# Princic-1837592/julia-raytracer

Hardware: AMD Instinct MI355X
Metric: Mrays/s + wall-clock render time, cornellbox 1280×720×256spp (higher is better)
Workload: dtype f32; 1 GPU; cornellbox path 1280x720x256spp; scene=cornellbox, sampler=path, width=1280, height=720, spp=256, bounces=8, batch=256, traversal=near, traversal_requested=auto, bvh=middle, parallelism=1 tile groups x 1 sample ranges + RCCL reduce

## Files before the change

### julia-raytracer_amd/csrc/jt_kernels.h

```cpp
#pragma once

#include <hip/hip_runtime.h>

#include <algorithm>

#include "jt_integrator.h"
#include "jt_launch.h"

namespace jtk {
using namespace jtd;

#ifndef JT_STAMPS
#define JT_STAMPS 0
#endif
#ifndef JT_NODE_REPEAT_NONE
#define JT_NODE_REPEAT_NONE 4
#endif
#ifndef JT_NODE_REPEAT
#define JT_NODE_REPEAT 3
#endif
#ifndef JT_FIRST_POP_NONE
#define JT_FIRST_POP_NONE 1
#endif
#ifndef JT_FIRST_POP
#define JT_FIRST_POP 2
#endif
template <int F>
constexpr int first_pops() { return !ft_none(F) && (F & FT_LINL) ? JT_FIRST_POP : JT_FIRST_POP_NONE; }
#ifndef JT_VOTE_P
#define JT_VOTE_P 3
#endif
#ifndef JT_VOTE_N
#define JT_VOTE_N 1
#endif
#ifndef JT_RAY_FROM_PATH
#define JT_RAY_FROM_PATH 1
#endif

__device__ __forceinline__ int lane_count(unsigned long long m) {
    return __builtin_popcount((unsigned)m) + __builtin_popcount((unsigned)(m >> 32));
}

__device__ __forceinline__ unsigned wave_sum(unsigned v) {
    for (int off = 32; off > 0; off >>= 1) v += __shfl_xor(v, off, 64);
    return v;
}

#ifndef JT_KARG_RELOAD
#define JT_KARG_RELOAD 1
#endif
template <int F>
__host__ __device__ constexpr bool karg_reload() {
    return JT_KARG_RELOAD && !mesh_env_quad_family(F);
}
template <class T>
__device__ __forceinline__ T karg(size_t off) {
    typedef __attribute__((address_space(4))) const char* kptr;
    kptr p = (kptr)__builtin_amdgcn_kernarg_segment_ptr();
    asm volatile("" : "+s"(p));
    return *(const __attribute__((address_space(4))) T*)(p + off);
}
#ifndef JT_KARG_SCENE
#define JT_KARG_SCENE 1
#endif
template <bool NCACHE, int F>
__host__ __device__ constexpr bool karg_scene() {
    return NCACHE && JT_KARG_SCENE && !mesh_family(F);
}
template <bool FROM_KARG>
__device__ __forceinline__ const DScene& shade_scene(const DScene& S) {
    if constexpr (FROM_KARG) {
        typedef __attribute__((address_space(4))) const char* kptr;
        kptr p = (kptr)__builtin_amdgcn_kernarg_segment_ptr();
        asm volatile("" : "+s"(p));
        return *(const DScene*)(const __attribute__((address_space(4))) DScene*)(p + offsetof(KArgs, S));
    } else {
        return S;
    }
}
#ifndef JT_KARG_PARAMS
#define JT_KARG_PARAMS 1
#endif
template <int SAMPLER, int F>
__host__ __device__ constexpr bool karg_params_on() {
    return JT_KARG_PARAMS && SAMPLER == 1 && !mesh_family(F);
}
template <bool FROM_KARG>
__device__ __forceinline__ const DParams& karg_params(const DParams& P) {
    if constexpr (FROM_KARG) {
        typedef __attribute__((address_space(4))) const char* kptr;
        kptr p = (kptr)__builtin_amdgcn_kernarg_segment_ptr();
        asm volatile("" : "+s"(p));
        return *(const DParams*)(const __attribute__((address_space(4))) DParams*)(p + offsetof(KArgs, P));
    } else {
        return P;
    }
}
#ifndef JT_KARG_SCENE_LDS
#define JT_KARG_SCENE_LDS 1
#endif
__device__ __forceinline__ DScene blob_scene(const DScene& S, const uint4* blob);
template <bool NCACHE, int RING, bool OVF, int F>
__device__ __forceinline__ DScene shade_scene_lds(const DScene& S0) {
    if constexpr (!NCACHE && JT_KARG_SCENE_LDS) {
        extern __shared__ uint4 dyn_lds[];
        const DScene& K = shade_scene<true>(S0);
        return blob_scene(K, dyn_lds + lds_stack_bytes(OVF, RING, K.stack_need) / 16);
    } else {
        return S0;
    }
}
#define JT_A(f) (karg_reload<F>() ? karg<decltype(DAccum::f)>(offsetof(KArgs, A) + offsetof(DAccum, f)) : A.f)
#define JT_SB (karg_reload<F>() ? karg<int>(offsetof(KArgs, s_begin)) : s_begin)
#define JT_SE (karg_reload<F>() ? karg<int>(offsetof(KArgs, s_end)) : s_end)


#ifndef JT_BAND_STRIP
#define JT_BAND_STRIP 16
#endif

#ifndef JT_ITEM_FIRST_POP
#define JT_ITEM_FIRST_POP 2
#endif
template <bool WIDE, int F>
__host__ __device__ constexpr bool item_first_pop() {
    return JT_ITEM_FIRST_POP == 1 || (JT_ITEM_FIRST_POP == 2 && !WIDE && !ft_none(F));
}
#ifndef JT_ITEM_COORDS
#define JT_ITEM_COORDS 1
#endif
template <int F>
__host__ __device__ constexpr bool item_coords() {
    return JT_ITEM_COORDS && !mesh_env_quad_family(F);
}
__device__ __forceinline__ int item_pixel(unsigned item, const DParams& P, int tiles_x) {
    const int t = (int)(item >> 6), l = (int)(item & 63u);
    return ((t / tiles_x) * 8 + (l >> 3)) * P.width + (t % tiles_x) * 8 + (l & 7);
}
template <int F>
__device__ __forceinline__ unsigned item_of(int ut, int l, int i, int j) {
    return item_coords<F>() ? item_encode(i, j) : (unsigned)(ut * 64 + l);
}
template <int F>
__device__ __forceinline__ int item_pixel_index(unsigned item, const DParams& P, int tiles_x) {
    return item_coords<F>() ? item_j(item) * P.width + item_i(item) : item_pixel(item, P, tiles_x);
}
template <int F>
__device__ __forceinline__ int item_slot(unsigned item, const DParams& P) {
    if constexpr (item_coords<F>()) return item_slot(item, (P.width + 7) >> 3, P.tile_offset, P.tile_stride_rcp);
    else {
        const float inv = __uint_as_float(__builtin_amdgcn_readfirstlane(__float_as_uint(1.0f / (float)P.tile_stride)));
        return launch_tile((int)(item >> 6), P.tile_offset, inv) * 64 + (int)(item & 63u);
    }
}
__device__ __forceinline__ float stream_weight(const DParams& P, int s) {
    return jl_rcp_weight((float)(((s - P.first) >> P.lk) + 1));
}

#if JT_STAMPS
#define JT_STAMP(x) x
#else
#define JT_STAMP(x)
#endif

template <int SAMPLER, int RING, bool OVF, int COUNT, int F, bool NCACHE, bool WIDE, bool ADAPT = false>
__device__ __forceinline__ void trace_body_items(const DScene& S0, const DParams& P0, int s_begin, int s_end,
                                                 const DAccum& A, int* stack) {
    const DScene& S = S0;
    const DParams& P = P0;
    static_assert(lane_lds(F), "the per-lane item body keeps the lane's sample index in LDS");
    constexpr int PB = push_bit(node_baked<OVF, NCACHE, WIDE, F>());
    const int lane = threadIdx.x & 63;
    const int oslot = (int)blockIdx.x * BLOCK + (int)threadIdx.x;
    if constexpr ((F & (FT_TEX | FT_ENV)) != 0) {
        for (int k = threadIdx.x; k < 512; k += BLOCK) tex_lut[k] = k < 256 ? S.srgb_lut[k] : S.byte_lut[k - 256];
        __syncthreads();
    }
    Counters cnt{0, 0, 0, 0};
    constexpr bool WC = !ft_none(F);
    unsigned w_paths = 0, w_rays = 0, w_lq = 0;
    __shared__ unsigned wave_cnt[WC ? 1 : (BLOCK / 64) * 4];
    unsigned* const wcnt = wave_cnt + (WC ? 0 : (threadIdx.x >> 6) * 4);
    if (!WC && lane < 3) wcnt[lane] = 0u;
    auto lds_count = [&](int k, bool c) {
        if (c) __hip_atomic_fetch_add(wcnt + k, 1u, __ATOMIC_RELAXED, __HIP_MEMORY_SCOPE_WORKGROUP);
    };
    __shared__ float acc_lds[acc_slots(F) * BLOCK];
    float* acc = acc_lds + threadIdx.x;
    int* const acc_i = reinterpret_cast<int*>(acc);
#if JT_STAMPS
    unsigned long long t_trav = 0, t_shade = 0, n_trav = 0, n_shade = 0, lanes_p = 0, lanes_n = 0, steps_p = 0, steps_n = 0;
    unsigned long long t_hit = 0, t_fin = 0, t_qb = 0, n_phit = 0, n_fin = 0, idle = 0, n_mph = 0, n_mty = 0, n_mid = 0;
    unsigned long long lanes_sh = 0, lanes_hit = 0, t_start = 0, n_start = 0, lanes_start = 0;
#endif
    const int tiles_x = (P.width + 7) / 8, tiles = launch_tiles(P);
    const int kstr = 1 << P.lk;
    const int nq = s_end - s_begin < kstr ? s_end - s_begin : kstr;
    unsigned xcc;
    asm volatile("s_getreg_b32 %0, hwreg(HW_REG_XCC_ID)" : "=s"(xcc));
    int band_k = 0;
    int ut = 0, uq = 0, bnext = 64;
    bool drained = false;
    unsigned item = ITEM_NONE;
    bool next_sample = false;
    Aov aov{acc, 0.0f, P.first, P.lk};
    Path st;
    st.pk = acc + acc_base_slots(F) * BLOCK;
    Trav T;
    T.sp = -1;
    T.nprim = 0;
    T.nxt = W_EMPTY;
    for (;;) {
        JT_STAMP(const unsigned long long ts0 = __builtin_amdgcn_s_memtime());
        bool start = next_sample;
        for (;;) {
            const unsigned long long needm = __builtin_amdgcn_ballot_w64(item == ITEM_NONE);
            if (!needm || drained) break;
            if (bnext >= 64) {
                const int band = (int)((xcc + (unsigned)band_k) & (NBANDS - 1));
                constexpr int STRIP = JT_BAND_STRIP;
                const int gx = tiles_x % P.tile_stride == 0 ? tiles_x / P.tile_stride : 0;
                const bool strips = STRIP > 1 && gx > 0;
                const int tiles_y = (P.height + 7) / 8;
                const int bt0 = strips ? band * tiles_y / NBANDS * gx : band * tiles / NBANDS;
                const int bn = strips ? (band + 1) * tiles_y / NBANDS * gx - bt0 : (band + 1) * tiles / NBANDS - bt0;
                unsigned unit = 0;
                if (lane == 0) unit = atomicAdd(JT_A(work) + band * BAND_STRIDE, 1u);
                unit = __builtin_amdgcn_readfirstlane(unit);
                if (unit >= (unsigned)bn * (unsigned)nq) {
                    if (++band_k >= NBANDS) drained = true;
                    continue;
                }
                uq = (int)(unit % (unsigned)nq);
                const int tu = (int)(unit / (unsigned)nq);
                int tile = bt0 + tu;
                if (strips) {
                    const int rows = bn / gx, sidx = tu / (STRIP * gx);
                    const int v = tu - sidx * STRIP * gx, h = rows - sidx * STRIP < STRIP ? rows - sidx * STRIP : STRIP;
                    tile = bt0 + (sidx * STRIP + v % h) * gx + v / h;
                }
                ut = tile * P.tile_stride + P.tile_offset;
                if constexpr (ADAPT) {
                    if (JT_A(frozen)[ut]) {
                        bnext = 64;
                        continue;
                    }
                }
                bnext = 0;
            }
            const int nneed = lane_count(needm), take = nneed < 64 - bnext ? nneed : 64 - bnext;
            const int rank = (int)__builtin_amdgcn_mbcnt_hi((unsigned)(needm >> 32), __builtin_amdgcn_mbcnt_lo((unsigned)needm, 0u));
            if (item == ITEM_NONE && rank < take) {
                const int l = bnext + rank;
                const int i = (ut % tiles_x) * 8 + (l & 7), j = (ut / tiles_x) * 8 + (l >> 3);
                if (i < P.width && j < P.height) {
                    item = item_of<F>(ut, l, i, j);
                    start = true;
                    const int s = JT_SB + uq;
                    acc_i[11 * BLOCK] = s;
                    const int pixel = j * P.width + i;
                    float4 im = make_float4(0, 0, 0, 0), al = im, nr = im;
                    int h = 0;
                    if (s - P.first >= kstr) {
                        if (P.lk == 0) {
                            im = JT_A(image)[pixel];
                            al = JT_A(albedo)[pixel];
                            nr = JT_A(normal)[pixel];
                            h = (int)JT_A(hits)[pixel];
                        } else {
                            const size_t o = (size_t)((s - P.first) & (kstr - 1)) * (size_t)JT_A(nslot) +
                                             (size_t)item_slot<F>(item, P);
                            im = JT_A(part_img)[o];
                            al = JT_A(part_alb)[o];
                            nr = JT_A(part_nrm)[o];
                            h = __float_as_int(al.w);
                        }
                    }
                    acc[0] = im.x;
                    acc[BLOCK] = im.y;
                    acc[2 * BLOCK] = im.z;
                    acc[3 * BLOCK] = im.w;
                    acc[4 * BLOCK] = al.x;
                    acc[5 * BLOCK] = al.y;
                    acc[6 * BLOCK] = al.z;
                    acc[7 * BLOCK] = nr.x;
                    acc[8 * BLOCK] = nr.y;
                    acc[9 * BLOCK] = nr.z;
                    acc_i[10 * BLOCK] = h;
                }
            }
            bnext += take;
        }
        next_sample = false;
        if (start) {
            const int sample = acc_i[11 * BLOCK];
            const int tpixel = item_coords<F>() ? 0 : item_pixel(item, P, tiles_x);
            if (!ft_none(F)) acc[12 * BLOCK] = stream_weight(P, sample);
            const DParams& P = karg_params<karg_params_on<SAMPLER, F>()>(P0);
            const int i = item_coords<F>() ? item_i(item) : tpixel % P.width;
            const int j = item_coords<F>() ? item_j(item) : tpixel / P.width;
            start_path<F>(P, i, j, item_coords<F>() ? j * P.width + i : tpixel, sample, st);
            query_start<WIDE>(S, T, st.o, st.d, -1, stack, 0, PB);
            if (!WC) lds_count(1, true);
            if constexpr (item_first_pop<WIDE, F>()) {
#pragma unroll
                for (int k = 0; k < first_pops<F>(); k++)
                    if (wants_node<WIDE>(T)) node_step_any<WIDE, RING, OVF, COUNT, NCACHE, F>(S, T, stack, oslot, cnt);
            }
        }
        if (WC) w_rays += lane_count(__builtin_amdgcn_ballot_w64(start));
#if JT_STAMPS
        const unsigned long long ts1 = __builtin_amdgcn_s_memtime();
        t_start += ts1 - ts0;
        n_start++;
        lanes_start += lane_count(__builtin_amdgcn_ballot_w64(start));
#endif
        if (__builtin_amdgcn_ballot_w64(item != ITEM_NONE) == 0) break;
        constexpr bool LSTEP = light_steps(SAMPLER, F);
        for (;;) {
            const bool wantp = T.nprim > 0;
            const bool wantn = wants_node<WIDE>(T);
            const bool waiting = query_done<WIDE>(T);
            const int np = lane_count(__builtin_amdgcn_ballot_w64(wantp));
            const int nn = lane_count(__builtin_amdgcn_ballot_w64(wantn));
            int nw = lane_count(__builtin_amdgcn_ballot_w64(waiting));
            const int nb = np + nn;
            if (LSTEP && !S.light_inline) {
                const bool wantl = waiting && st.phase == PH_LIGHT;
                const int nl = lane_count(__builtin_amdgcn_ballot_w64(wantl));
                if (nl > 0 && (nl >= P.light_lanes || nb == 0)) {
                    bool c_lq = false, c_ray = false;
                    if (wantl && rerun_tie<WIDE>(S, T, st.o, st.d, S.lights[st.li].instance, stack, PB)) {
                    } else if (wantl) {
                        if (light_hit<F>(S, P, st, query_hit(T))) {
                            st.phase = PH_FINISH;
                        } else if (st.phase == PH_LIGHT) {
                            if (WC) c_lq = true;
                            else lds_count(2, true);
                            query_start<WIDE>(S, T, st.o, st.d, S.lights[st.li].instance, stack, 0, PB);
                        } else {
                            if (WC) c_ray = true;
                            else lds_count(1, true);
                            query_start<WIDE>(S, T, st.o, st.d, -1, stack, 0, PB);
                        }
                    }
                    if (WC) {
                        w_lq += lane_count(__builtin_amdgcn_ballot_w64(c_lq));
                        w_rays += lane_count(__builtin_amdgcn_ballot_w64(c_ray));
                    }
                    continue;
                }
                nw -= nl;
            }
            if (nb == 0 || nw >= (nb + nw < P.wait_lanes ? nb + nw : P.wait_lanes)) break;
#if JT_STAMPS
            n_trav++;
            idle += 64 - lane_count(__builtin_amdgcn_ballot_w64(item != ITEM_NONE));
            if (np * JT_VOTE_P >= nn * JT_VOTE_N) { steps_p++; lanes_p += np; } else { steps_n++; lanes_n += nn; }
#endif
            if (JT_RAY_FROM_PATH && !(F & FT_XFORM)) {
                T.lo = st.o;
                T.ld = st.d;
            }
            if (np * JT_VOTE_P >= nn * JT_VOTE_N) {
                if (T.nprim > 0) prim_step<COUNT, F>(S, T, cnt);
            } else {
                constexpr int NREP = ft_none(F) ? JT_NODE_REPEAT_NONE : JT_NODE_REPEAT;
#pragma unroll
                for (int k = 0; k < NREP; k++)
                    if (wants_node<WIDE>(T)) node_step_any<WIDE, RING, OVF, COUNT, NCACHE, F>(S, T, stack, oslot, cnt);
            }
        }
#if JT_STAMPS
        const unsigned long long ts2 = __builtin_amdgcn_s_memtime();
        t_trav += ts2 - ts1;
        n_shade++;
        lanes_sh += lane_count(__builtin_amdgcn_ballot_w64(query_done<WIDE>(T)));
        {
            int mid = -1, mt = -1;
            if (query_done<WIDE>(T) && st.phase == PH_SCENE && T.h_inst >= 0) {
                mid = S.inst_shade[T.h_inst].material;
                mt = (F & FT_MAT) ? S.materials[mid].type : (int)M_MATTE;
            }
            if (__builtin_amdgcn_ballot_w64(mt >= 0)) {
                n_mph++;
                lanes_hit += lane_count(__builtin_amdgcn_ballot_w64(mt >= 0));
                for (int ty = 0; ty <= (int)M_GLTFPBR; ty++) n_mty += __builtin_amdgcn_ballot_w64(mt == ty) ? 1u : 0u;
                bool counted = mt < 0;
                for (;;) {
                    const unsigned long long m = __builtin_amdgcn_ballot_w64(!counted);
                    if (!m) break;
                    const int v = __shfl(mid, __ffsll((long long)m) - 1);
                    counted = counted || mid == v;
                    n_mid++;
                }
            }
        }
        unsigned long long ts3 = ts2, ts4 = ts2;
#endif
        constexpr bool LINL = (F & (FT_LINL | FT_NOIL)) != 0;
        {
            const bool tie = query_done<WIDE>(T) && (T.nh & (TIE_SEEN | REF_RERUN)) == TIE_SEEN &&
                             !(LSTEP && st.phase == PH_FINISH);
            if (S.order_flip && __builtin_amdgcn_ballot_w64(tie))
                if (tie) rerun_tie<WIDE>(S, T, st.o, st.d, SAMPLER == 1 && !LINL && st.phase == PH_LIGHT ? S.lights[st.li].instance : -1, stack, PB);
        }
        bool c_path = false, c_lq = false, c_ray = false;
        unsigned n_inl = 0;
        if (query_done<WIDE>(T)) {
            const DParams& P = karg_params<karg_params_on<SAMPLER, F>()>(P0);
            const DScene SL = shade_scene_lds<NCACHE, RING, OVF, F>(S0);
            const DScene& S = NCACHE ? shade_scene<karg_scene<NCACHE, F>()>(S0) : SL;
            bool alive = true;
            const bool light = SAMPLER == 1 && !LINL && st.phase == PH_LIGHT;
            bool done;
            if (LSTEP && st.phase == PH_FINISH) done = true;
            else if (light) done = light_hit<F>(S, P, st, query_hit(T));
            else if (SAMPLER == 2) done = naive_hit<F>(S, P, st, query_hit(T), aov, cnt.shades);
            else done = path_hit<F>(S, P, st, query_hit(T), aov, cnt.shades);
            bool chained = false;
            if (SAMPLER == 1 && !done && st.phase == PH_LIGHT && chains_inline(F, S)) {
                unsigned nlq = 0;
                chained = true;
                done = light_chain<WIDE, RING, OVF, COUNT, NCACHE, F>(S, P, st, T, stack, oslot, cnt, [&] {
                    if (WC) nlq++;
                    else lds_count(2, true);
                });
                if (WC) n_inl += nlq;
            }
#if JT_STAMPS
            ts3 = __builtin_amdgcn_s_memtime();
            n_phit++;
#endif
            if (done) {
                if (WC) c_path = true;
                else lds_count(0, true);
                v3 radiance = st.radiance<F>();
                if (!all_finite(radiance)) radiance = V3(0, 0, 0);
                const float mr = max3(radiance);
                if (mr > P.clamp) radiance = radiance * (P.clamp / mr);
                const float w = aov.w<F>();
                const float omw = 1 - w;
                const bool hit = st.flag(F_HIT);
                const bool env = !hit && !P.envhidden && S.nenvs != 0;
                const v4 target = (hit || env) ? V4(radiance.x, radiance.y, radiance.z, 1) : V4(0, 0, 0, 0);
                if (!hit) aov_update<F>(aov, env ? V3(1, 1, 1) : V3(0, 0, 0), -st.d);
                acc[0] = acc[0] * omw + target.x * w;
                acc[BLOCK] = acc[BLOCK] * omw + target.y * w;
                acc[2 * BLOCK] = acc[2 * BLOCK] * omw + target.z * w;
                acc[3 * BLOCK] = acc[3 * BLOCK] * omw + target.w * w;
                if (hit || env) acc_i[10 * BLOCK] += 1;
                alive = false;
                T.sp = -1;
                const int sample = acc_i[11 * BLOCK];
                if (sample + kstr >= JT_SE) {
                    const int pixel = item_pixel_index<F>(item, P, tiles_x);
                    const float4 im = make_float4(acc[0], acc[BLOCK], acc[2 * BLOCK], acc[3 * BLOCK]);
                    if (P.lk == 0) {
                        JT_A(image)[pixel] = im;
                        JT_A(albedo)[pixel] = make_float4(acc[4 * BLOCK], acc[5 * BLOCK], acc[6 * BLOCK], 0.0f);
                        JT_A(normal)[pixel] = make_float4(acc[7 * BLOCK], acc[8 * BLOCK], acc[9 * BLOCK], 0.0f);
                        JT_A(hits)[pixel] = (long long)acc_i[10 * BLOCK];
                    } else {
                        const size_t o = (size_t)((sample - P.first) & (kstr - 1)) * (size_t)JT_A(nslot) +
                                         (size_t)item_slot<F>(item, P);
                        JT_A(part_img)[o] = im;
                        JT_A(part_alb)[o] = make_float4(acc[4 * BLOCK], acc[5 * BLOCK], acc[6 * BLOCK], __int_as_float(acc_i[10 * BLOCK]));
                        JT_A(part_nrm)[o] = make_float4(acc[7 * BLOCK], acc[8 * BLOCK], acc[9 * BLOCK], 0.0f);
                    }
                    item = ITEM_NONE;
                } else {
                    acc_i[11 * BLOCK] = sample + kstr;
                    next_sample = true;
                }
            }
#if JT_STAMPS
            ts4 = __builtin_amdgcn_s_memtime();
            if (__builtin_amdgcn_ballot_w64(done)) n_fin++;
#endif
            if (alive) {
                if (SAMPLER == 1 && !LINL && st.phase == PH_LIGHT) {
                    if (WC) c_lq = true;
                    else lds_count(2, true);
                    query_start<WIDE>(S, T, st.o, st.d, S.lights[st.li].instance, stack, 0, PB);
                } else {
                    if (WC) c_ray = true;
                    else lds_count(1, true);
                    if (SAMPLER == 1 && chain_dinv_once<WIDE, OVF, NCACHE, F>() && __builtin_amdgcn_ballot_w64(!chained) == 0)
                        query_restart<F>(S, T, st.o, st.d, stack, PB);
                    else query_start<WIDE>(S, T, st.o, st.d, -1, stack, 0, PB);
                }
#pragma unroll
                for (int k = 0; k < first_pops<F>(); k++)
                    if (wants_node<WIDE>(T)) node_step_any<WIDE, RING, OVF, COUNT, NCACHE, F>(S, T, stack, oslot, cnt);
            }
        }
#if JT_STAMPS
        const unsigned long long ts5 = __builtin_amdgcn_s_memtime();
        t_shade += ts5 - ts2;
        t_hit += ts3 - ts2;
        t_fin += ts4 - ts3;
        t_qb += ts5 - ts4;
#endif
        if (WC) {
            w_paths += lane_count(__builtin_amdgcn_ballot_w64(c_path));
            w_lq += lane_count(__builtin_amdgcn_ballot_w64(c_lq));
            w_rays += lane_count(__builtin_amdgcn_ballot_w64(c_ray));
            if (SAMPLER == 1 && chains_inline(F, S)) w_lq += __builtin_amdgcn_readfirstlane(wave_sum(n_inl));
        }
    }
#if JT_STAMPS
    if (lane == 0) {
        unsigned long long* dbg = A.counters + 8;
        const unsigned long long v[24] = {t_trav, t_shade, n_trav,  n_shade, lanes_p, lanes_n,  steps_p, steps_n,
                                          0,      t_hit,   t_fin,   t_qb,    0,       n_phit,   n_fin,   idle,
                                          n_mph,  n_mty,   n_mid,   lanes_sh, lanes_hit, t_start, n_start, lanes_start};
        for (int k = 0; k < 24; k++) atomicAdd(dbg + k, v[k]);
    }
#endif
    const unsigned wv[3] = {w_paths, w_rays, w_lq};
    unsigned v[7] = {0u, 0u, 0u, cnt.nodes, cnt.instances, cnt.prims, COUNT ? cnt.shades : 0u};
#pragma unroll
    for (int k = 0; k < 7; k++) {
        unsigned sum = k < 3 ? (WC ? wv[k] : wcnt[k]) : wave_sum(v[k]);
        if (lane == 0 && sum) atomicAdd(&A.counters[k], (unsigned long long)sum);
    }
}

#ifndef JT_WAVES
#define JT_WAVES 0
#endif
#ifndef JT_WAVES_NONE
#define JT_WAVES_NONE 5
#endif
#if JT_WAVES > 0
#define JT_WAVES_PER_EU __attribute__((amdgpu_waves_per_eu(JT_WAVES, JT_WAVES)))
#define JT_WAVES_PER_EU_F(F) \
    __attribute__((amdgpu_waves_per_eu(ft_none(F) ? JT_WAVES_NONE : JT_WAVES, ft_none(F) ? JT_WAVES_NONE : JT_WAVES)))
#else
#define JT_WAVES_PER_EU
#define JT_WAVES_PER_EU_F(F)
#endif

__device__ __forceinline__ DScene blob_scene(const DScene& S, const uint4* blob) {
    DScene L = S;
    L.nodes = reinterpret_cast<const DNode*>(blob + S.o_nodes);
    L.wnodes = reinterpret_cast<const DWide*>(blob + S.o_wnodes);
    L.prims = reinterpret_cast<const float4*>(blob + S.o_prims);
    L.inst_trav = reinterpret_cast<const DInstTrav*>(blob + S.o_inst_trav);
    L.inst_blas = reinterpret_cast<const int4*>(blob + S.o_inst_blas);
    L.inst_shade = reinterpret_cast<const DInstShade*>(blob + S.o_inst_shade);
    L.shapes = reinterpret_cast<const DShape*>(blob + S.o_shapes);
    L.pos = reinterpret_cast<const float4*>(blob + S.o_pos);
    L.nrm = reinterpret_cast<const float4*>(blob + S.o_nrm);
    L.tc = reinterpret_cast<const float2*>(blob + S.o_tc);
    L.col = reinterpret_cast<const float4*>(blob + S.o_col);
    L.elems = reinterpret_cast<const int4*>(blob + S.o_elems);
    L.enrm = reinterpret_cast<const float4*>(blob + S.o_enrm);
    L.enrm_id = reinterpret_cast<const float4*>(blob + S.o_enrm_id);
    L.materials = reinterpret_cast<const DMaterial*>(blob + S.o_materials);
    L.lights = reinterpret_cast<const DLight*>(blob + S.o_lights);
    L.light_hit = reinterpret_cast<const int4*>(blob + S.o_light_hit);
    L.light_elems = reinterpret_cast<const float4*>(blob + S.o_light_elems);
    L.cdf = reinterpret_cast<const float*>(blob + S.o_cdf);
    return L;
}

__device__ __forceinline__ void bake_nodes(const DScene& S, uint4* blob) {
    uint4* const nodes = blob + S.o_nodes;
    const int nnodes = (S.o_wnodes - S.o_nodes) >> 1;
    for (int k = threadIdx.x; k < nnodes; k += BLOCK) {
        uint4& b = nodes[2 * k + 1];
        const BakedNode bn = bake_node(b.w, (int)b.z, k < S.tlas_nnodes ? T_TLAS : T_BLAS);
        b.z = bn.e0;
        b.w = bn.meta;
    }
}

template <int SAMPLER, int RING, bool OVF, int COUNT, int F, bool WIDE, bool ADAPT>
__global__ __launch_bounds__(BLOCK) JT_WAVES_PER_EU void trace_kernel(DScene S, DParams P, int s_begin, int s_end, DAccum A) {
    __shared__ int lds_stack[RING * BLOCK];
    trace_body_items<SAMPLER, RING, OVF, COUNT, F, true, WIDE, ADAPT>(S, P, s_begin, s_end, A, lds_stack + threadIdx.x);
}

template <int SAMPLER, int RING, bool OVF, int COUNT, int F, bool WIDE, bool ADAPT>
__global__ __launch_bounds__(BLOCK) JT_WAVES_PER_EU_F(F) void trace_kernel_lds(DScene S, DParams P, int s_begin, int s_end, DAccum A) {
    extern __shared__ uint4 dyn_lds[];
    uint4* blob = dyn_lds + lds_stack_bytes(OVF, RING, S.stack_need) / 16;
    for (int k = threadIdx.x; k < S.blob_n16; k += BLOCK) blob[k] = S.blob[k];
    __syncthreads();
    if constexpr (node_baked<OVF, false, WIDE, F>()) {
        bake_nodes(S, blob);
        __syncthreads();
    }
    const DScene L = blob_scene(S, blob);
    trace_body_items<SAMPLER, RING, OVF, COUNT, F, false, WIDE, ADAPT>(L, P, s_begin, s_end, A, reinterpret_cast<int*>(dyn_lds) + threadIdx.x);
}

template <int SAMPLER, int RING, bool OVF, int COUNT, int F, bool LDSK, bool WIDE, bool ADAPT>
hipError_t launch_t(const DScene& S, const DParams& P, int s0, int s1, const DAccum& A, hipStream_t st, int cus) {
    const long long units = (long long)launch_tiles(P) * std::min(s1 - s0, 1 << P.lk);
    const int want = (int)std::min<long long>((units + BLOCK / 64 - 1) / (BLOCK / 64), 1 << 30);
    if (want == 0) return hipSuccess;
    int per_cu = 0;
    hipError_t e;
    if constexpr (LDSK) {
        if (S.blob_n16 > 0) {
        const size_t lds = lds_stack_bytes(OVF, RING, S.stack_need) + (size_t)S.blob_n16 * 16;
        constexpr auto kl = &trace_kernel_lds<SAMPLER, RING, OVF, COUNT, F, WIDE, ADAPT>;
        const void* k = (const void*)kl;
        if ((e = hipFuncSetAttribute(k, hipFuncAttributeMaxDynamicSharedMemorySize, (int)lds)) != hipSuccess) return e;
        if (hipOccupancyMaxActiveBlocksPerMultiprocessor(&per_cu, k, BLOCK, lds) != hipSuccess || per_cu < 1) per_cu = 1;
        const int nwg = std::min(want, std::min(per_cu, 8) * cus);
        hipLaunchKernelGGL(kl, dim3(nwg), dim3(BLOCK), lds, st, S, P, s0, s1, A);
        return hipGetLastError();
        }
    }
    constexpr auto kh = &trace_kernel<SAMPLER, RING, OVF, COUNT, F, WIDE, ADAPT>;
    const void* k = (const void*)kh;
    if (hipOccupancyMaxActiveBlocksPerMultiprocessor(&per_cu, k, BLOCK, 0) != hipSuccess || per_cu < 1) per_cu = 1;
    const int nwg = std::min(want, std::min(per_cu, 8) * cus);
    hipLaunchKernelGGL(kh, dim3(nwg), dim3(BLOCK), 0, st, S, P, s0, s1, A);
    return hipGetLastError();
}

template <int ID, int SAMPLER, int COUNT, bool ADAPT>
hipError_t launch_cfg(const DScene& S, const DParams& P, int s0, int s1, const DAccum& A, hipStream_t st, int cus) {
    using C = LaunchConfig<ID>;
    return launch_t<SAMPLER, C::ring, C::ovf, COUNT, C::feat, C::lds, C::wide, ADAPT>(S, P, s0, s1, A, st, cus);
}

}
```

### julia-raytracer_amd/csrc/jt_push.h

```cpp
#pragma once

#if defined(__HIPCC__) || defined(__CUDACC__)
#define JT_PUSH_HD __host__ __device__ inline
#else
#define JT_PUSH_HD inline
#endif

namespace jtk {

constexpr int PUSH_SLOTS = 4;
constexpr unsigned PUSH_T_INST = 1u, PUSH_SNAP_NONE = 63u << 24;

struct PushPlan {
    int npush;
    int first, step;
    unsigned tag;
    bool leaf;
    int slot[PUSH_SLOTS];
    unsigned value[PUSH_SLOTS];
};

JT_PUSH_HD PushPlan push_plan(unsigned meta, int start, unsigned type, bool blas, int negmask, int sp) {
    PushPlan p;
    const bool internal = (meta >> 24) != 0;
    const int num = (int)(meta & 0xffffu);
    const bool neg = ((negmask >> (int)((meta >> 16) & 3u)) & 1) != 0;
    p.npush = internal ? 2 : blas ? 0 : num;
    p.first = internal ? (neg ? start + 1 : start) : start + num - 1;
    p.step = internal && !neg ? 1 : -1;
    p.tag = (internal ? type << 30 : PUSH_T_INST << 30) | PUSH_SNAP_NONE;
    p.leaf = blas && !internal;
    const int last = (p.npush > 1 ? p.npush : 1) - 1;
    const unsigned e0 = p.tag | (unsigned)p.first;
    for (int j = 0; j < PUSH_SLOTS; j++) {
        const int k = j < last ? j : last;
        p.slot[j] = sp + k;
        p.value[j] = e0 + (unsigned)(p.step * k);
    }
    return p;
}

constexpr unsigned BAKE_AXIS_SET = 3u;
constexpr int BAKE_MASK_BIT = 8;
constexpr unsigned BAKE_LEAF = 1u << 27;

struct BakedNode {
    unsigned e0, meta;
};
JT_PUSH_HD BakedNode bake_node(unsigned meta, int start, unsigned level) {
    const bool internal = (meta >> 24) != 0;
    const bool blas = level != 0u;
    const unsigned num = meta & 0xffffu;
    const unsigned tag = (internal ? level << 30 : PUSH_T_INST << 30) | PUSH_SNAP_NONE;
    const unsigned npush = internal ? 2u : blas ? 0u : (num < (unsigned)PUSH_SLOTS ? num : (unsigned)PUSH_SLOTS);
    const unsigned last = (npush > 1u ? npush : 1u) - 1u;
    BakedNode b;
    b.e0 = internal || !blas ? tag | (unsigned)start : (unsigned)start;
    b.meta = num | (internal ? (meta >> 16) & 3u : BAKE_AXIS_SET) << 16 | npush << 24 | (!internal && blas ? BAKE_LEAF : 0u) |
             last << 28 | (last ? 1u : 0u) << 30;
    return b;
}
JT_PUSH_HD unsigned add_absdiff(unsigned a, unsigned b, unsigned c) {
#if defined(__HIP_DEVICE_COMPILE__)
    unsigned r;
    __asm__("v_sad_u32 %0, %1, %2, %3" : "=v"(r) : "v"(a), "v"(b), "v"(c));
    return r;
#else
    return c + (a > b ? a - b : b - a);
#endif
}
JT_PUSH_HD PushPlan push_plan_baked(unsigned e0, unsigned meta, int negmask, int sp) {
    PushPlan p;
    p.npush = (int)((meta >> 24) & 7u);
    p.first = 0;
    p.step = 0;
    p.tag = 0u;
    p.leaf = (meta & BAKE_LEAF) != 0;
    const unsigned neg = ((unsigned)negmask >> ((meta >> 16) & 3u)) & 1u;
    const unsigned last = (meta >> 28) & 3u;
    const unsigned nlast = last * neg;
    for (int j = 0; j < PUSH_SLOTS; j++) {
        const unsigned k = j == 1 ? (meta >> 30) & 1u : (unsigned)j < last ? (unsigned)j : last;
        p.slot[j] = sp + (int)k;
        p.value[j] = j == 0 ? e0 + nlast : add_absdiff(nlast, k, e0);
    }
    return p;
}

}
```

### julia-raytracer_amd/csrc/jt_traverse.h

```cpp
#pragma once

#include <hip/hip_runtime.h>

#include "jt_device.h"
#include "jt_launch.h"
#include "jt_push.h"

#ifndef JT_CHILD_PRETEST
#define JT_CHILD_PRETEST 1
#endif

namespace jtk {
using namespace jtd;


struct Hit {
    int inst, elem;
    float u, v, t;
    bool hit;
};
struct Counters {
    unsigned nodes, instances, prims, shades;
};

struct Trav {
    v3 wo, wd, wdinv;
    v3 lo, ld, ldinv;
    float tmax;
    int sp;
    int low;
    int inst_space;
    int negmask;
    int cur_inst, cur_kind;
    int prim, nprim;
    int h_inst, h_elem;
    float h_u, h_v;
    int nh;
    unsigned nxt;
};

#ifndef JT_TIE_RERUN
#define JT_TIE_RERUN 1
#endif
constexpr int TIE_SEEN = 1 << 8, REF_RERUN = 1 << 9, NH_COUNT = 63;
__device__ __forceinline__ int query_flip(const DScene& S, const Trav& T, int pb = 0) {
    return ((T.nh & REF_RERUN) ? 0 : S.order_flip) | pb;
}
__device__ __forceinline__ void hit_count(Trav& T, float t) {
    T.nh = (T.nh + ((T.nh & NH_COUNT) < NH_COUNT ? 1 : 0)) | (JT_TIE_RERUN && t == T.tmax ? TIE_SEEN : 0);
}

#ifndef JT_NODE_BAKE
#define JT_NODE_BAKE 1
#endif
#ifndef JT_NODE_READ16
#define JT_NODE_READ16 0
#endif
template <bool OVF, bool NCACHE, bool WIDE, int F>
__host__ __device__ constexpr bool node_baked() {
    return JT_NODE_BAKE && !OVF && !NCACHE && !WIDE && ft_none(F);
}
__host__ __device__ constexpr int push_bit(bool baked) { return baked ? BAKE_MASK_BIT : 0; }

__device__ __forceinline__ int neg_mask(v3 d, int flip) {
    return ((d.x < 0 ? 1 : 0) | (d.y < 0 ? 2 : 0) | (d.z < 0 ? 4 : 0)) ^ flip;
}

__device__ __forceinline__ void world_ray(const DScene& S, Trav& T, int pb = 0) {
    T.lo = T.wo;
    T.ld = T.wd;
    T.ldinv = T.wdinv;
    T.negmask = neg_mask(T.wd, query_flip(S, T, pb));
    T.inst_space = 0;
}

__device__ __forceinline__ Hit query_hit(const Trav& T) {
    return Hit{T.h_inst, T.h_elem, T.h_u, T.h_v, T.tmax, T.h_inst >= 0};
}

__device__ __forceinline__ bool query_busy(const Trav& T) { return T.sp > 0 || T.nprim > 0; }
template <bool WIDE>
__device__ __forceinline__ bool wants_node(const Trav& T) {
    return T.nprim == 0 && (T.sp > 0 || (WIDE && T.nxt != W_EMPTY));
}
template <bool WIDE>
__device__ __forceinline__ bool query_done(const Trav& T) {
    return (T.sp | T.nprim) == 0 && (!WIDE || T.nxt == W_EMPTY);
}

__device__ __forceinline__ void query_ray(Trav& T, v3 o, v3 d) {
    T.wo = o;
    T.wd = d;
    T.wdinv = V3(jl_rcp(d.x), jl_rcp(d.y), jl_rcp(d.z));
    T.lo = o;
    T.ld = d;
    T.ldinv = T.wdinv;
}
__device__ __forceinline__ void query_reset(Trav& T, int nh) {
    T.tmax = __builtin_inff();
    T.nh = nh;
    T.h_inst = -1;
    T.h_elem = -1;
    T.h_u = 0;
    T.h_v = 0;
    T.nprim = 0;
    T.prim = 0;
    T.cur_inst = -1;
    T.cur_kind = KIND_TRI;
    T.inst_space = 0;
}
__device__ __forceinline__ void query_begin(const DScene& S, Trav& T, v3 o, v3 d, unsigned root, int* stack, int rerun = 0,
                                            int pb = 0) {
    query_ray(T, o, d);
    query_reset(T, rerun);
    T.negmask = neg_mask(d, (rerun ? 0 : S.order_flip) | pb);
    stack[0] = (int)root;
    T.sp = 1;
    T.low = 0;
    T.nxt = W_EMPTY;
}
__device__ __forceinline__ void query_begin_wide(const DScene& S, Trav& T, v3 o, v3 d, unsigned root_word, int rerun = 0) {
    query_ray(T, o, d);
    query_reset(T, rerun);
    T.negmask = neg_mask(d, rerun ? 0 : S.order_flip);
    T.sp = 0;
    T.low = 0;
    T.nxt = root_word;
}
constexpr unsigned WROOT_SCENE = 0u;
__device__ __forceinline__ unsigned wroot_instance(int inst) { return W_LEAF | W_INST | (unsigned)inst; }
template <bool WIDE>
__device__ __forceinline__ void query_start(const DScene& S, Trav& T, v3 o, v3 d, int inst, int* stack, int rerun = 0,
                                            int pb = 0) {
    if (WIDE) query_begin_wide(S, T, o, d, inst < 0 ? WROOT_SCENE : wroot_instance(inst), rerun);
    else query_begin(S, T, o, d, inst < 0 ? ((T_TLAS << 30) | SNAP_NONE) : ((T_INST << 30) | SNAP_NONE | (unsigned)inst), stack, rerun, pb);
}
template <int F>
__device__ __forceinline__ void query_restart(const DScene& S, Trav& T, v3 o, v3 d, int* stack, int pb = 0) {
    T.wo = o;
    T.wd = d;
    T.lo = o;
    T.ld = d;
    T.ldinv = T.wdinv;
    query_reset(T, 0);
    if (F & FT_XFORM) T.negmask = neg_mask(d, S.order_flip | pb);
    stack[0] = (int)((T_TLAS << 30) | SNAP_NONE);
    T.sp = 1;
    T.low = 0;
    T.nxt = W_EMPTY;
}
constexpr int INST_LEAF_ROOT = 1 << 30;
template <bool WIDE>
__device__ __forceinline__ bool rerun_tie(const DScene& S, Trav& T, v3 o, v3 d, int inst, int* stack, int pb = 0) {
    if (!JT_TIE_RERUN || (T.nh & (TIE_SEEN | REF_RERUN)) != TIE_SEEN || S.order_flip == 0) return false;
    if (inst >= 0 && (S.inst_blas[inst].w & INST_LEAF_ROOT)) return false;
    query_start<WIDE>(S, T, o, d, inst, stack, REF_RERUN, pb);
    return true;
}

template <bool XF>
__device__ __forceinline__ void enter_instance(const DScene& S, Trav& T, unsigned inst, const int4& ib, int pb = 0) {
    if (!XF || ib.y) {
        if (XF && T.inst_space) world_ray(S, T, pb);
    } else {
        const DInstTrav it = S.inst_trav[inst];
        const fr3 inv = frame_from(it.i0, it.i1, it.i2);
        T.lo = transform_point(inv, T.wo);
        T.ld = transform_vector(inv, T.wd);
        T.ldinv = V3(jl_rcp(T.ld.x), jl_rcp(T.ld.y), jl_rcp(T.ld.z));
        T.negmask = neg_mask(T.ld, query_flip(S, T, pb));
        T.inst_space = 1;
    }
    T.cur_inst = (int)inst;
    T.cur_kind = ib.z;
}

template <int F>
__device__ __forceinline__ void tri_pair(const DScene& S, Trav& T, int k) {
    const float4* r = S.prims + 5 * (T.prim + (k >> 1));
    const float4 r0 = r[0], r1 = r[1], r2 = r[2], r3 = r[3], r4 = r[4];
    const PrimHit p1 = intersect_triangle_pre(T.lo, T.ld, ray_eps, V3(r0.x, r0.z, r1.x), V3(r1.z, r2.x, r2.z),
                                              V3(r3.x, r3.z, r4.x));
    const PrimHit p2 = intersect_triangle_pre(T.lo, T.ld, ray_eps, V3(r0.y, r0.w, r1.y), V3(r1.w, r2.y, r2.w),
                                              V3(r3.y, r3.w, r4.y));
    if (tri_hit_before(p1, T.tmax)) {
        hit_count(T, p1.t);
        T.h_inst = T.cur_inst;
        T.h_elem = __float_as_int(r4.z);
        T.h_u = p1.u;
        T.h_v = p1.v;
        T.tmax = p1.t;
    }
    if (T.nprim >= k + 2 && tri_hit_before(p2, T.tmax)) {
        hit_count(T, p2.t);
        T.h_inst = T.cur_inst;
        T.h_elem = __float_as_int(r4.w);
        T.h_u = p2.u;
        T.h_v = p2.v;
        T.tmax = p2.t;
    }
}
template <int COUNT, int F>
__device__ __forceinline__ void prim_step(const DScene& S, Trav& T, Counters& cnt) {
    if (!(F & FT_QUAD) || T.cur_kind == KIND_TRI) {
        tri_pair<F>(S, T, 0);
        const bool more = T.nprim > 2;
        if (__builtin_amdgcn_ballot_w64(more)) {
            if (more) tri_pair<F>(S, T, 2);
        }
        const int n = T.nprim < 4 ? T.nprim : 4;
        if (COUNT) cnt.prims += n;
        T.prim += 2;
        T.nprim -= n;
        return;
    }
    if (COUNT) cnt.prims++;
    const float4* r = S.prims + 4 * T.prim;
    const float4 a = r[0], b = r[1], c = r[2], d = r[3];
    const PrimHit p = intersect_quad(T.lo, T.ld, ray_eps, T.tmax, xyz(a), xyz(b), xyz(c), xyz(d), d.w != 0.0f);
    if (p.hit) {
        hit_count(T, p.t);
        T.h_inst = T.cur_inst;
        T.h_elem = __float_as_int(a.w);
        T.h_u = p.u;
        T.h_v = p.v;
        T.tmax = p.t;
    }
    T.prim += 1;
    T.nprim -= 1;
}

template <int RING, bool OVF>
__device__ __forceinline__ void st_push(const DScene& S, Trav& T, int* stack, int pixel, unsigned e) {
    if (OVF) {
        if (T.sp - T.low == S.ring) {
            S.ovf[(size_t)pixel * S.ovf_stride + T.low] = stack[(T.low & (S.ring - 1)) * BLOCK];
            T.low += 1;
        }
        stack[(T.sp & (S.ring - 1)) * BLOCK] = (int)e;
    } else {
        stack[T.sp * BLOCK] = (int)e;
    }
    T.sp += 1;
}
template <int RING, bool OVF>
__device__ __forceinline__ unsigned st_pop(const DScene& S, Trav& T, const int* stack, int pixel) {
    T.sp -= 1;
    if (OVF) {
        const unsigned r = (unsigned)__hip_atomic_load(stack + (T.sp & (S.ring - 1)) * BLOCK, __ATOMIC_RELAXED,
                                                       __HIP_MEMORY_SCOPE_WORKGROUP);
        if (T.sp < T.low) {
            T.low = T.sp;
            return (unsigned)S.ovf[(size_t)pixel * S.ovf_stride + T.sp];
        }
        return r;
    }
    return (unsigned)stack[T.sp * BLOCK];
}

template <int RING, bool OVF, int COUNT, bool NCACHE, int F>
__device__ __forceinline__ void node_step(const DScene& S, Trav& T, int* stack, int pixel, Counters& cnt) {
    constexpr bool XF = (F & FT_XFORM) != 0;
    constexpr bool BAKED = node_baked<OVF, NCACHE, false, F>();
    constexpr int PB = push_bit(BAKED);
    const unsigned e = st_pop<RING, OVF>(S, T, stack, pixel);
    unsigned type = e >> 30, idx = e & IDX_MASK;
    if (type == T_INST) {
        if (COUNT) cnt.instances++;
        const int4 ib = S.inst_blas[idx];
        enter_instance<XF>(S, T, idx, ib, PB);
        type = T_BLAS;
        idx = (unsigned)ib.x;
    } else if (XF && type == T_TLAS && T.inst_space) {
        world_ray(S, T, PB);
    }
    const bool blas = type == T_BLAS;
    if (COUNT) cnt.nodes++;
    const unsigned snap = (e >> 24) & 63u;
    float4 nb;
    if (NCACHE) {
        nb = S.nodes[idx].b;
        __asm__("" : "+v"(nb.x), "+v"(nb.y), "+v"(nb.z), "+v"(nb.w));
        if (snap == 63u || snap != (unsigned)(T.nh & NH_COUNT))
            if (!intersect_bbox(T.lo, T.ldinv, ray_eps, T.tmax, S.nodes[idx].a, nb)) return;
    } else {
        DNode nd = S.nodes[idx];
        if (JT_NODE_READ16 && BAKED) __asm__("" : "+v"(nd.b.x), "+v"(nd.b.y), "+v"(nd.b.z), "+v"(nd.b.w));
        if (!intersect_bbox(T.lo, T.ldinv, ray_eps, T.tmax, nd.a, nd.b)) return;
        nb = nd.b;
    }
    const unsigned meta = __float_as_uint(nb.w);
    const int start = __float_as_int(nb.z);
    const int num = (int)(meta & 0xffffu);
    if (!OVF && !(JT_CHILD_PRETEST && NCACHE)) {
        if constexpr (BAKED) {
            const PushPlan p = push_plan_baked((unsigned)start, meta, T.negmask, T.sp);
            int* const top = stack + T.sp * BLOCK;
#pragma unroll
            for (int j = 0; j < PUSH_SLOTS; j++) top[(p.slot[j] - T.sp) * BLOCK] = (int)p.value[j];
            T.sp += p.npush;
            T.prim = p.leaf ? start : T.prim;
            T.nprim = p.leaf ? num : T.nprim;
            return;
        }
        const PushPlan p = push_plan(meta, start, type, blas, T.negmask, T.sp);
#pragma unroll
        for (int j = 0; j < PUSH_SLOTS; j++) stack[p.slot[j] * BLOCK] = (int)p.value[j];
        T.sp += p.npush;
        T.prim = p.leaf ? start : T.prim;
        T.nprim = p.leaf ? num : T.nprim;
        return;
    }
    if (meta >> 24) {
        const int axis = (int)((meta >> 16) & 0xffu);
        const bool neg = (T.negmask >> axis) & 1;
        const unsigned tag = type << 30 | SNAP_NONE;
        const unsigned c_second = (unsigned)(neg ? start + 1 : start), c_first = (unsigned)(neg ? start : start + 1);
        if (JT_CHILD_PRETEST && NCACHE) {
            const DNode n0 = S.nodes[c_second];
            const DNode n1 = S.nodes[c_first];
            const bool k0 = intersect_bbox(T.lo, T.ldinv, ray_eps, T.tmax, n0.a, n0.b);
            const bool k1 = intersect_bbox(T.lo, T.ldinv, ray_eps, T.tmax, n1.a, n1.b);
            if (COUNT) cnt.nodes += (k0 ? 0 : 1) + (k1 ? 0 : 1);
            const unsigned ptag = type << 30 | (unsigned)(T.nh & NH_COUNT) << 24;
            if (k0) st_push<RING, OVF>(S, T, stack, pixel, ptag | c_second);
            if (k1) st_push<RING, OVF>(S, T, stack, pixel, ptag | c_first);
        } else {
            st_push<RING, OVF>(S, T, stack, pixel, tag | c_second);
            st_push<RING, OVF>(S, T, stack, pixel, tag | c_first);
        }
    } else if (!blas) {
        for (int k = num - 1; k >= 0; k--)
            st_push<RING, OVF>(S, T, stack, pixel, (T_INST << 30) | SNAP_NONE | (unsigned)(start + k));
    } else {
        T.prim = start;
        T.nprim = num;

    }
}

__device__ __forceinline__ int wide_slot(unsigned flips, int k) {
    const int p = (k >> 1) ^ (int)(flips & 1u);
    return 2 * p + ((k & 1) ^ (int)((flips >> (p ? 2 : 1)) & 1u));
}
__device__ __forceinline__ unsigned wide_word(const uint4& r3, int slot) {
    return slot == 0 ? r3.x : slot == 1 ? r3.y : slot == 2 ? r3.z : r3.w;
}
__device__ __forceinline__ float deq(float o, unsigned w, int sh, float s) {
    return __builtin_fmaf((float)((w >> sh) & 255u), s, o);
}
__device__ __forceinline__ void wide_box(const float4& r0, const uint4& r1, const uint4& r2, float sx, float sy,
                                         float sz, int c, float4& a, float4& b) {
    const int sh = 8 * c;
    a = make_float4(deq(r0.x, r1.x, sh, sx), deq(r0.x, r1.y, sh, sx), deq(r0.y, r1.z, sh, sy), deq(r0.y, r1.w, sh, sy));
    b = make_float4(deq(r0.z, r2.x, sh, sz), deq(r0.z, r2.y, sh, sz), 0.0f, 0.0f);
}
template <int F>
__device__ __forceinline__ void wide_take(Trav& T, unsigned w) {
    const bool leaf = (w & (W_LEAF | W_INST)) == W_LEAF;
    T.prim = leaf ? (int)(w & W_START) : T.prim;
    T.nprim = leaf ? (int)((w >> 28) & 3u) + 1 : T.nprim;

    T.nxt = leaf ? T.nxt : w;
}
template <int RING, bool OVF, int COUNT, int F>
__device__ __forceinline__ void wide_visit(const DScene& S, Trav& T, int* stack, int pixel, Counters& cnt, unsigned idx) {
    if (COUNT) cnt.nodes++;
    const DWide& rec = S.wnodes[idx];
    const float4 r0 = rec.r0;
    const uint4 r1 = rec.r1, r2 = rec.r2, r3 = rec.r3;
    const unsigned meta = __float_as_uint(r0.w);
    const float sx = __uint_as_float((meta & 255u) << 23), sy = __uint_as_float(((meta >> 8) & 255u) << 23),
                sz = __uint_as_float(((meta >> 16) & 255u) << 23);
    unsigned hits = 0;
#pragma unroll
    for (int c = 0; c < 4; c++) {
        float4 a, b;
        wide_box(r0, r1, r2, sx, sy, sz, c, a, b);
        const bool pass = intersect_bbox(T.lo, T.ldinv, ray_eps, T.tmax, a, b);
        if (wide_word(r3, c) != W_EMPTY && pass) hits |= 1u << c;
    }
    if (!hits) return;
    const unsigned ax = meta >> 24;
    const unsigned flips = ((T.negmask >> (ax & 3u)) & 1u ? 0u : 1u) | ((T.negmask >> ((ax >> 2) & 3u)) & 1u ? 0u : 2u) |
                           ((T.negmask >> ((ax >> 4) & 3u)) & 1u ? 0u : 4u);
    unsigned vm = 0;
#pragma unroll
    for (int k = 0; k < 4; k++) vm |= ((hits >> wide_slot(flips, k)) & 1u) << k;
    const int k0 = __builtin_ctz(vm);
    const unsigned rest = vm & (vm - 1u);
    if (rest) st_push<RING, OVF>(S, T, stack, pixel, flips << 28 | rest << 24 | idx);
    wide_take<F>(T, wide_word(r3, wide_slot(flips, k0)));
}
template <int RING, bool OVF, int COUNT, int F>
__device__ __forceinline__ void node_step_wide(const DScene& S, Trav& T, int* stack, int pixel, Counters& cnt) {
    constexpr bool XF = (F & FT_XFORM) != 0;
    unsigned w = T.nxt;
    if (w == W_EMPTY) {
        const unsigned e = st_pop<RING, OVF>(S, T, stack, pixel);
        const unsigned idx = e & IDX_MASK;
        if (!(e >> 31)) {
            const unsigned m = (e >> 24) & 15u;
            const unsigned rest = m & (m - 1u);
            if (rest) st_push<RING, OVF>(S, T, stack, pixel, (e & ~(15u << 24)) | rest << 24);
            if (XF && T.inst_space && idx < (unsigned)S.tlas_wnodes) world_ray(S, T);
            w = reinterpret_cast<const unsigned*>(S.wnodes + idx)[12 + wide_slot((e >> 28) & 7u, __builtin_ctz(m))];
            if ((w & (W_LEAF | W_INST)) == W_LEAF) {
                wide_take<F>(T, w);
                return;
            }
        } else {
            w = W_LEAF | W_INST | ((e >> 24) & 3u) << 28 | idx;
        }
    } else {
        T.nxt = W_EMPTY;
    }
    if (w & W_LEAF) {
        const unsigned inst = w & W_START, n1 = (w >> 28) & 3u;
        if (n1) st_push<RING, OVF>(S, T, stack, pixel, W_LEAF | (n1 - 1u) << 24 | (inst + 1u));
        if (COUNT) cnt.instances++;
        const int4 ib = S.inst_blas[inst];
        enter_instance<XF>(S, T, inst, ib);
        w = (unsigned)ib.x;
    }
    wide_visit<RING, OVF, COUNT, F>(S, T, stack, pixel, cnt, w);
}
template <bool WIDE, int RING, bool OVF, int COUNT, bool NCACHE, int F>
__device__ __forceinline__ void node_step_any(const DScene& S, Trav& T, int* stack, int pixel, Counters& cnt) {
    if (WIDE) node_step_wide<RING, OVF, COUNT, F>(S, T, stack, pixel, cnt);
    else node_step<RING, OVF, COUNT, NCACHE, F>(S, T, stack, pixel, cnt);
}

template <int COUNT, int F>
__device__ __forceinline__ void inst_leaf_query(const DScene& S, Trav& T, v3 o, v3 d, v3 dinv, int negmask, int inst,
                                                Counters& cnt) {
    constexpr bool XF = (F & FT_XFORM) != 0;
    constexpr int PB = push_bit(node_baked<false, false, false, F>());
    T.wo = o;
    T.wd = d;
    T.wdinv = dinv;
    T.lo = o;
    T.ld = d;
    T.ldinv = dinv;
    query_reset(T, 0);
    T.negmask = negmask;
    T.sp = 0;
    T.low = 0;
    T.nxt = W_EMPTY;
    if (COUNT) cnt.instances++;
    const int4 ib = S.inst_blas[inst];
    enter_instance<XF>(S, T, (unsigned)inst, ib, PB);
    if (COUNT) cnt.nodes++;
    const DNode nd = S.nodes[ib.x];
    const bool pass = intersect_bbox(T.lo, T.ldinv, ray_eps, T.tmax, nd.a, nd.b);
    T.prim = pass ? __float_as_int(nd.b.z) : 0;
    T.nprim = pass ? (int)(__float_as_uint(nd.b.w) & 0xffffu) : 0;
}

}
```

Baseline: 13580 Mrays/s.

## Copy instance BLAS roots into node array so instance entries index them directly

During node baking, each instance's BLAS root node is copied into a per-instance slot appended after the node array. TLAS leaf pushes are rebased so instance entries point at these slots, and the baked traversal path skips the inst_blas lookup and enter_instance call, only recording the current instance. This removes a dependent load per instance entry but relies on the blob layout having room at o_inst_trav. It also assumes no transform is needed on instance entry, which holds only for the transform-free baked path.

```diff
diff --git a/julia-raytracer_amd/csrc/jt_kernels.h b/julia-raytracer_amd/csrc/jt_kernels.h
--- a/julia-raytracer_amd/csrc/jt_kernels.h
+++ b/julia-raytracer_amd/csrc/jt_kernels.h
@@ -569,11 +569,24 @@
 __device__ __forceinline__ void bake_nodes(const DScene& S, uint4* blob) {
     uint4* const nodes = blob + S.o_nodes;
     const int nnodes = (S.o_wnodes - S.o_nodes) >> 1;
+    const int iroot0 = JT_INST_ROOTS ? instance_root_base(S.o_nodes, S.o_inst_trav) : 0;
     for (int k = threadIdx.x; k < nnodes; k += BLOCK) {
         uint4& b = nodes[2 * k + 1];
-        const BakedNode bn = bake_node(b.w, (int)b.z, k < S.tlas_nnodes ? T_TLAS : T_BLAS);
+        const BakedNode bn = bake_node(b.w, (int)b.z, k < S.tlas_nnodes ? T_TLAS : T_BLAS, iroot0);
         b.z = bn.e0;
         b.w = bn.meta;
+    }
+    if (JT_INST_ROOTS) {
+        const int ninst = (S.o_inst_blas - S.o_inst_trav) >> 2;
+        for (int i = threadIdx.x; i < ninst; i += BLOCK) {
+            const uint4* const root = S.blob + S.o_nodes + 2 * (int)S.blob[S.o_inst_blas + i].x;
+            uint4 b = root[1];
+            const BakedNode bn = bake_node(b.w, (int)b.z, T_BLAS);
+            b.z = bn.e0;
+            b.w = bn.meta;
+            nodes[2 * (iroot0 + i)] = root[0];
+            nodes[2 * (iroot0 + i) + 1] = b;
+        }
     }
 }
 
diff --git a/julia-raytracer_amd/csrc/jt_push.h b/julia-raytracer_amd/csrc/jt_push.h
--- a/julia-raytracer_amd/csrc/jt_push.h
+++ b/julia-raytracer_amd/csrc/jt_push.h
@@ -47,10 +47,11 @@
 struct BakedNode {
     unsigned e0, meta;
 };
-JT_PUSH_HD BakedNode bake_node(unsigned meta, int start, unsigned level) {
+JT_PUSH_HD BakedNode bake_node(unsigned meta, int start, unsigned level, int iroot0 = 0) {
     const bool internal = (meta >> 24) != 0;
     const bool blas = level != 0u;
     const unsigned num = meta & 0xffffu;
+    if (!internal && !blas) start += iroot0;
     const unsigned tag = (internal ? level << 30 : PUSH_T_INST << 30) | PUSH_SNAP_NONE;
     const unsigned npush = internal ? 2u : blas ? 0u : (num < (unsigned)PUSH_SLOTS ? num : (unsigned)PUSH_SLOTS);
     const unsigned last = (npush > 1u ? npush : 1u) - 1u;
@@ -87,4 +88,11 @@
     return p;
 }
 
+JT_PUSH_HD int instance_root_base(int o_nodes, int o_inst_trav) { return (o_inst_trav - o_nodes + 1) >> 1; }
+constexpr unsigned PUSH_IDX_MASK = (1u << 24) - 1;
+JT_PUSH_HD unsigned instance_root_entry(int iroot0, int inst) {
+    return PUSH_T_INST << 30 | PUSH_SNAP_NONE | (unsigned)(iroot0 + inst);
 }
+JT_PUSH_HD int instance_of_entry(int iroot0, unsigned e) { return (int)(e & PUSH_IDX_MASK) - iroot0; }
+
+}
diff --git a/julia-raytracer_amd/csrc/jt_traverse.h b/julia-raytracer_amd/csrc/jt_traverse.h
--- a/julia-raytracer_amd/csrc/jt_traverse.h
+++ b/julia-raytracer_amd/csrc/jt_traverse.h
@@ -61,6 +61,12 @@
     return JT_NODE_BAKE && !OVF && !NCACHE && !WIDE && ft_none(F);
 }
 __host__ __device__ constexpr int push_bit(bool baked) { return baked ? BAKE_MASK_BIT : 0; }
+#ifndef JT_INST_ROOTS
+#define JT_INST_ROOTS 1
+#endif
+__device__ __forceinline__ int inst_root_base(const DScene& S, int pb) {
+    return JT_INST_ROOTS && pb ? instance_root_base(S.o_nodes, S.o_inst_trav) : 0;
+}
 
 __device__ __forceinline__ int neg_mask(v3 d, int flip) {
     return ((d.x < 0 ? 1 : 0) | (d.y < 0 ? 2 : 0) | (d.z < 0 ? 4 : 0)) ^ flip;
@@ -132,6 +138,7 @@
 template <bool WIDE>
 __device__ __forceinline__ void query_start(const DScene& S, Trav& T, v3 o, v3 d, int inst, int* stack, int rerun = 0,
                                             int pb = 0) {
+    if (JT_INST_ROOTS && pb && inst >= 0) inst += inst_root_base(S, pb);
     if (WIDE) query_begin_wide(S, T, o, d, inst < 0 ? WROOT_SCENE : wroot_instance(inst), rerun);
     else query_begin(S, T, o, d, inst < 0 ? ((T_TLAS << 30) | SNAP_NONE) : ((T_INST << 30) | SNAP_NONE | (unsigned)inst), stack, rerun, pb);
 }
@@ -265,7 +272,10 @@
     constexpr int PB = push_bit(BAKED);
     const unsigned e = st_pop<RING, OVF>(S, T, stack, pixel);
     unsigned type = e >> 30, idx = e & IDX_MASK;
-    if (type == T_INST) {
+    if constexpr (BAKED && JT_INST_ROOTS) {
+        if (COUNT) cnt.instances += type == T_INST ? 1u : 0u;
+        T.cur_inst = type == T_INST ? instance_of_entry(inst_root_base(S, PB), e) : T.cur_inst;
+    } else if (type == T_INST) {
         if (COUNT) cnt.instances++;
         const int4 ib = S.inst_blas[idx];
         enter_instance<XF>(S, T, idx, ib, PB);
@@ -448,10 +458,17 @@
     T.low = 0;
     T.nxt = W_EMPTY;
     if (COUNT) cnt.instances++;
-    const int4 ib = S.inst_blas[inst];
-    enter_instance<XF>(S, T, (unsigned)inst, ib, PB);
+    int root;
+    if constexpr (JT_INST_ROOTS && PB != 0) {
+        T.cur_inst = inst;
+        root = inst_root_base(S, PB) + inst;
+    } else {
+        const int4 ib = S.inst_blas[inst];
+        enter_instance<XF>(S, T, (unsigned)inst, ib, PB);
+        root = ib.x;
+    }
     if (COUNT) cnt.nodes++;
-    const DNode nd = S.nodes[ib.x];
+    const DNode nd = S.nodes[root];
     const bool pass = intersect_bbox(T.lo, T.ldinv, ray_eps, T.tmax, nd.a, nd.b);
     T.prim = pass ? __float_as_int(nd.b.z) : 0;
     T.nprim = pass ? (int)(__float_as_uint(nd.b.w) & 0xffffu) : 0;
```

Result: faster. 13940 Mrays/s, median of 6 (+2.7%).
